# Vegeta2020/SE-SSD

Hardware: NVIDIA H100
Metric: frames_per_sec (higher is better)
Workload: dtype f32

## Files before the change

### include/sessd_b200_lab.h

```cpp
#ifndef SESSD_B200_LAB_H
#define SESSD_B200_LAB_H

#include "sessd_b200.h"

#ifdef __cplusplus
extern "C" {
#endif

int sessd_bev_conv_h2(const float *d_in, const void *d_weight_h2, int cout_pad, const float *d_scale,
                      const float *d_shift, const float *d_residual, float *d_out, const sessd_conv_desc *desc,
                      const float *d_amax_in, float *d_amax_out, void *stream);
int sessd_bev_deconv_h2(const float *d_in, const void *d_weight_h2, int cout_pad, const float *d_scale,
                        const float *d_shift, const float *d_residual, float *d_out, int batch, int in_h, int in_w,
                        int cin, int cout, int relu, const float *d_amax_in, float *d_amax_out, void *stream);

int sessd_bev_conv_p2_profile(const void *d_in_planes, const float *d_in_info, const void *d_weight_h2, int cout_pad,
                              const float *d_scale, const float *d_shift, const float *d_residual, const float *d_resid_info,
                              float gain, float shift_max, float *d_out_f32, void *d_out_planes, float *d_out_info,
                              const sessd_conv_desc *desc, const int *d_items, long long *d_prof, void *stream);
int sessd_bev_deconv_p2_profile(const void *d_in_planes, const float *d_in_info, const void *d_weight_h2, int cout_pad,
                                const float *d_scale, const float *d_shift, const float *d_residual, const float *d_resid_info,
                                float gain, float shift_max, float *d_out_f32, void *d_out_planes, float *d_out_info, int batch,
                                int in_h, int in_w, int cin, int cout, int relu, const int *d_items, long long *d_prof,
                                void *stream);

int sessd_bev_conv_p2_loads(const void *d_in_planes, const float *d_in_info, const void *d_weight_h2, int cout_pad,
                            const float *d_scale, const float *d_shift, const float *d_residual, const float *d_resid_info,
                            float gain, float shift_max, float *d_out_f32, void *d_out_planes, float *d_out_info,
                            const sessd_conv_desc *desc, const int *d_items, int smem_a, long long *d_prof, void *stream);

int sessd_bev_p2_plan(const sessd_conv_desc *desc, int deconv, int cout_pad, int split, int smem_a, int *plan);

#ifdef __cplusplus
}
#endif
#endif
```

### se-ssd_b200/csrc/bevconv_p2.cuh

```cuda
#pragma once
#include <cuda_fp16.h>

#include "tc_common.cuh"

namespace sessd {

constexpr int kP2TileU = 8, kP2TileV = 16;
constexpr int kP2MaxCopies = 6, kP2MaxRowsV = 18;
constexpr int kP2BStages = 6, kP2MaxBStages = 12;
constexpr int kP2MmaWarps = 8;
constexpr int kP2PatchWarp = 8, kP2WeightWarp = 9;
constexpr int kP2Threads = 320;
constexpr int kP2ThreadsRegA = 384, kP2RegsConsumer = 232, kP2RegsProducer = 40;
static_assert(2 * (kP2RegsConsumer - 168) <= 168 - kP2RegsProducer, "the consumers take what the producers release");
constexpr int kP2MaxSmem = 227 * 1024;
constexpr int kP2Chunk = 32;
constexpr int kP2ItemsHeader = 32;
enum { kP2Planes = 0, kP2SplitF16 = 1 };
enum { kP2NoProbe = 0, kP2ProbeClocks = 1, kP2ProbeLoads = 2 };

struct P2Params {
    int batch, cin, cout;
    int in_stride;
    int out_h, out_w;
    int grid_u, grid_v;
    int u_is_x;
    int out_stride, nclass;
    int cls_ntaps[4], cls_off_u[4], cls_off_v[4];
    int tap_copy[4][9], tap_row[4][9], tap_w[4][9];
    int ncopies, rows_v, pitch_u;
    int copy_u[kP2MaxCopies], copy_v[kP2MaxCopies];
    int copy_bytes, patch_bytes, npatch;
    int load_bytes, staging_bytes;
    int bring_bytes;
    int out_info_scale;
    const float *in_amax;
    int relu, n_tile, nblocks;
    int bstages, bstage_bytes;
    int tiles_u, tiles_v, tiles, total;
    int cls_order[4];
    const float *in_info;
    const float *resid_info;
    float gain, shift_max;
    float *out_info;
    long long out_plane_stride;
    const int *items;
    long long *prof;
};

// ... 78 lines not shown
        }
}

template <bool PROFILE>
__device__ __forceinline__ long long p2_tick() {
    if constexpr (PROFILE) return clock64();
    return 0;
}
template <bool PROFILE>
__device__ __forceinline__ void p2_tock(long long &clk, long long t0) {
    if constexpr (PROFILE) clk += clock64() - t0;
}

__device__ __forceinline__ void p2_split_patch(const P2Params &p, const unsigned char *staging, unsigned char *planes, float s_in, int ctid) {
    const int rows = p.rows_v * kP2TileU;
    const int copy_in = p.staging_bytes / p.ncopies;
    const int items = p.ncopies * rows * 4;
    for (int i = ctid; i < items; i += kP2MmaWarps * 32) {
        const int j = i & 3, r = (i >> 2) % rows, c = (i >> 2) / rows;
        unsigned char *hi = planes + 2 * c * p.copy_bytes + r * 64 + ((j ^ ((r >> 1) & 3)) << 4);
        const float4 *src = reinterpret_cast<const float4 *>(staging + c * copy_in + r * 128 + j * 32);
        const float4 a = src[0], b = src[1];
        const float x[8] = {a.x * s_in, a.y * s_in, a.z * s_in, a.w * s_in, b.x * s_in, b.y * s_in, b.z * s_in, b.w * s_in};
        __align__(16) __half h[8], l[8];
#pragma unroll
        for (int t = 0; t < 8; ++t) { h[t] = __float2half_rn(x[t]); l[t] = __float2half_rn(x[t] - __half2float(h[t])); }
        *reinterpret_cast<uint4 *>(hi) = *reinterpret_cast<const uint4 *>(h);
        *reinterpret_cast<uint4 *>(hi + p.copy_bytes) = *reinterpret_cast<const uint4 *>(l);
    }
    asm volatile("fence.proxy.async.shared::cta;\n" ::: "memory");
    asm volatile("bar.sync 1, %0;\n" ::"n"(kP2MmaWarps * 32) : "memory");
}

template <int NT, int MODE, bool REGA = false, int PROBE = kP2NoProbe>
__global__ void __launch_bounds__(REGA ? kP2ThreadsRegA : kP2Threads, 1) bev_conv_p2_kernel(const __grid_constant__ CUtensorMap map_a,
                                                                   const __grid_constant__ CUtensorMap map_b,
                                                                   const float *__restrict__ scale, const float *__restrict__ shift,
                                                                   const float *__restrict__ resid, float *__restrict__ out_f32,
                                                                   __half *__restrict__ out_planes, P2Params p) {
    static_assert(!REGA || MODE == kP2Planes, "register-fed A reads the TMA-written planes");
    constexpr bool PROFILE = PROBE != kP2NoProbe, LOADS_ONLY = PROBE == kP2ProbeLoads;
    extern __shared__ unsigned char smem_raw[];
    unsigned char *tiles = (unsigned char *)(((uintptr_t)smem_raw + 1023) & ~(uintptr_t)1023);
    unsigned char *patches = tiles + p.bring_bytes;
    unsigned char *staging = patches + p.npatch * p.patch_bytes;
    uint64_t *bars = (uint64_t *)(staging + p.npatch * p.staging_bytes);
    uint64_t *patch_full = bars, *patch_empty = bars + 2, *b_full = bars + 4, *b_empty = bars + 4 + kP2MaxBStages;
    uint32_t *s_aoff = (uint32_t *)(b_empty + kP2MaxBStages);
    float *s_scale = (float *)(((uintptr_t)(s_aoff + 4 * 9) + 15) & ~(uintptr_t)15), *s_shift = s_scale + p.cout;

    const int warp = threadIdx.x >> 5, lane = threadIdx.x & 31;
    if (threadIdx.x == kP2PatchWarp * 32) prefetch_tensormap(&map_a);
    if (threadIdx.x == kP2WeightWarp * 32) prefetch_tensormap(&map_b);
    const int nchunks = p.cin / kP2Chunk;
    const int nitems = p2_item_count(p);
    const uint32_t b_plane_bytes = (uint32_t)p.n_tile * 64u;

    if (threadIdx.x == 0) {
        for (int s = 0; s < 2; ++s) { mbar_init(&patch_full[s], 1); mbar_init(&patch_empty[s], kP2MmaWarps); }
        for (int s = 0; s < p.bstages; ++s) { mbar_init(&b_full[s], 1); mbar_init(&b_empty[s], kP2MmaWarps); }
        asm volatile("fence.mbarrier_init.release.cluster;\n" ::: "memory");
    }
    for (int idx = threadIdx.x; idx < p.nclass * 9; idx += blockDim.x) {
        const int c = idx / 9, t = idx - c * 9;
        s_aoff[idx] = REGA ? (uint32_t)p.tap_row[c][t] : (uint32_t)((2 * p.tap_copy[c][t] * p.copy_bytes + p.tap_row[c][t] * 512) >> 4);
    }
    for (int n = threadIdx.x; n < p.cout; n += blockDim.x) {
        s_scale[n] = scale ? __ldg(scale + n) : 1.f;
        s_shift[n] = shift ? __ldg(shift + n) : 0.f;
    }
    __syncthreads();
    long long clk[kP2ProfWords] = {};
    const long long t_start = p2_tick<PROFILE>();
    long long *prof_rec = PROFILE ? p.prof + (size_t)blockIdx.x * kP2ProfWords : nullptr;

    if (warp >= kP2MmaWarps) {
        if constexpr (REGA) setmaxnreg_dec<kP2RegsProducer>();
        if (warp == kP2PatchWarp) {
            int pb = 0;
            uint32_t pph = 0;
            const uint32_t patches_u32 = smem_u32(patches);
            for (int k = blockIdx.x; k < nitems; k += gridDim.x) {
                const P2Item it = p2_decode(p, p2_item(p, k));
                const int bu = it.u0 * p.in_stride, bv = it.v0 * p.in_stride;
                for (int cc = 0; cc < nchunks; ++cc) {
                    { const long long t0 = p2_tick<PROFILE>(); mbar_wait<REGA>(&patch_empty[pb], pph ^ 1u); p2_tock<PROFILE>(clk[kProfPatchEmpty], t0); }
                    if (elect_one()) {
                        mbar_expect_tx(&patch_full[pb], (uint32_t)p.load_bytes);
                        if constexpr (MODE == kP2Planes) {
                            uint32_t dst = patches_u32 + (uint32_t)(pb * p.patch_bytes);
                            for (int c = 0; c < p.ncopies; ++c, dst += 2u * (uint32_t)p.copy_bytes) {
                                const int cu = bu + p.copy_u[c], cv = bv + p.copy_v[c];
                                tma_load_5d(dst, &map_a, &patch_full[pb], cc * kP2Chunk, cu, cv, it.b, 0);
                                tma_load_5d(dst + (uint32_t)p.copy_bytes, &map_a, &patch_full[pb], cc * kP2Chunk, cu, cv, it.b, 1);
                            }
                        } else {
                            const uint32_t copy_in = (uint32_t)(p.staging_bytes / p.ncopies);
                            uint32_t dst = smem_u32(staging) + (uint32_t)(pb * p.staging_bytes);
                            for (int c = 0; c < p.ncopies; ++c, dst += copy_in)
                                tma_load_5d(dst, &map_a, &patch_full[pb], cc * kP2Chunk, bu + p.copy_u[c], bv + p.copy_v[c], it.b, 0);
                        }
                    }
                    __syncwarp();
                    if (++pb == p.npatch) { pb = 0; pph ^= 1u; }
                }
            }
            if constexpr (PROFILE)
                if (lane == 0) {
                    prof_rec[kProfPatchEmpty] = clk[kProfPatchEmpty];
                    prof_rec[kProfPatchTotal] = clock64() - t_start;
                }
        } else if (warp == kP2WeightWarp) {
            int S = 0;
            uint32_t bph = 0;
            for (int k = blockIdx.x; k < nitems; k += gridDim.x) {
                const P2Item it = p2_decode(p, p2_item(p, k));
                for (int cc = 0; cc < nchunks; ++cc)
                    for (int tap = 0; tap < it.ntaps; ++tap) {
// ... 24 lines not shown
        const uint32_t patch_lo = desc_lo(smem_u32(patches)) + a_rows;
        const uint32_t plane_lo = b_plane_bytes >> 4;
        const uint32_t copy_lo = (uint32_t)(p.copy_bytes >> 4), patch_sz = (uint32_t)(p.patch_bytes >> 4);
        const uint32_t a_row = (uint32_t)((wg * 8 + wq * 2 + ((lane >> 3) & 1)) * p.pitch_u + (lane & 7)), a_chunk = (uint32_t)(lane >> 4);
        const uint32_t patches_u32 = smem_u32(patches);
        float amax_in = 0.f, s_in = 1.f;
        if constexpr (MODE == kP2Planes) { amax_in = __ldg(p.in_info); s_in = __ldg(p.in_info + 1); }
        if constexpr (MODE == kP2SplitF16) if (p.in_amax) { amax_in = __ldg(p.in_amax); s_in = pow2_scale_for_bound(amax_in); }
        const float inv_sa = 1.f / s_in;
        float bound = amax_in * p.gain + p.shift_max;
        if (p.resid_info) bound += __ldg(p.resid_info);
        const float s_out = pow2_scale_for_bound(bound);
        if (blockIdx.x == 0 && threadIdx.x == 0 && p.out_info && p.out_info_scale) p.out_info[1] = s_out;
        float vmax = 0.f;
        const int per_cls = p.nblocks * p.tiles;
        int S = 0, pb = 0;
        uint32_t bph = 0, pph = 0;
        for (int k = blockIdx.x; k < nitems; k += gridDim.x) {
            const long long t_item = p2_tick<PROFILE>();
            const int g = p2_item(p, k);
            const int cls = p.cls_order[g / per_cls];
            const int ntaps = p.cls_ntaps[cls];
            const uint32_t *aoff = s_aoff + cls * 9;
            float acc[NT];
#pragma unroll
            for (int i = 0; i < NT; ++i) acc[i] = 0.f;
            int prevS = -1, prev_pb = -1;
            bool first = true;
            if constexpr (REGA) {
                uint32_t frag[2][16];
                int tap = 0;
                uint32_t pbase = 0;
                auto load_frags = [&](uint32_t *fa) {
                    if (tap == 0) {
                        { const long long t0 = p2_tick<PROFILE>(); mbar_wait<REGA>(&patch_full[pb], pph); p2_tock<PROFILE>(clk[kProfPatchFull], t0); }
                        pbase = patches_u32 + (uint32_t)(pb * p.patch_bytes);
                    }
                    if constexpr (!LOADS_ONLY) {
                        const uint32_t r = a_row + aoff[tap];
                        const uint32_t a_hi = pbase + r * 64u + ((a_chunk ^ ((r >> 1) & 3u)) << 4), a_lo = a_hi + (uint32_t)p.copy_bytes;
                        ldsm_x4(fa, a_hi);
                        ldsm_x4(fa + 4, a_hi ^ 32u);
                        ldsm_x4(fa + 8, a_lo);
                        ldsm_x4(fa + 12, a_lo ^ 32u);
                    }
                };
                auto step_ra = [&](const uint32_t *fa, uint32_t *fn, bool more) {
                    { const long long t0 = p2_tick<PROFILE>(); mbar_wait<REGA>(&b_full[S], bph); p2_tock<PROFILE>(clk[kProfBFull], t0); }
                    const uint64_t db_lo = kDescSw64Hi | (uint64_t)(tiles_lo + (uint32_t)(S * (p.bstage_bytes >> 4)));
                    const uint64_t db_hi = db_lo + (uint64_t)plane_lo;
                    if constexpr (!LOADS_ONLY) {
                        wgmma_fence();
                        p2_wgmma_ra<2 * NT>(acc, fa, db_lo, first ? 0u : 1u);
                        p2_wgmma_ra<2 * NT>(acc, fa + 4, db_lo + 2, 1u);
                        wgmma_commit();
                    }
                    first = false;
                    if constexpr (PROFILE) ++clk[kProfSteps];
                    { const long long t0 = p2_tick<PROFILE>(); wgmma_wait<1>(); p2_tock<PROFILE>(clk[kProfMmaWait], t0); }
                    if (lane == 0 && prevS >= 0) mbar_arrive(&b_empty[prevS]);
                    prevS = S;
                    if (++S == p.bstages) { S = 0; bph ^= 1u; }
                    if (++tap == ntaps) {
                        tap = 0;
                        if (lane == 0) mbar_arrive(&patch_empty[pb]);
                        if (++pb == p.npatch) { pb = 0; pph ^= 1u; }
                    }
                    if (more) load_frags(fn);
                    if constexpr (!LOADS_ONLY) {
                        wgmma_fence();
                        p2_wgmma_ra<NT>(acc, fa + 8, db_hi, 1u);
                        p2_wgmma_ra<NT>(acc, fa + 12, db_hi + 2, 1u);
                        wgmma_commit();
                    }
                };
                const int nsteps = nchunks * ntaps;
                load_frags(frag[0]);
#pragma unroll 1
                for (int st = 0; st + 1 < nsteps; st += 2) { step_ra(frag[0], frag[1], true); step_ra(frag[1], frag[0], st + 2 < nsteps); }
                if (nsteps & 1) step_ra(frag[0], frag[1], false);
            } else {
                for (int cc = 0; cc < nchunks; ++cc) {
                    { const long long t0 = p2_tick<PROFILE>(); mbar_wait(&patch_full[pb], pph); p2_tock<PROFILE>(clk[kProfPatchFull], t0); }
                    if constexpr (MODE == kP2SplitF16)
                        p2_split_patch(p, staging + pb * p.staging_bytes, patches + pb * p.patch_bytes, s_in, threadIdx.x);
                    const uint32_t pbase = patch_lo + (uint32_t)pb * patch_sz;
#pragma unroll 1
                    for (int tap = 0; tap < ntaps; ++tap) {
                        { const long long t0 = p2_tick<PROFILE>(); mbar_wait(&b_full[S], bph); p2_tock<PROFILE>(clk[kProfBFull], t0); }
                        if constexpr (!LOADS_ONLY) {
                            const uint64_t da_hi = kDescSw64Hi | (uint64_t)(pbase + aoff[tap]);
                            const uint64_t da_lo = da_hi + (uint64_t)copy_lo;
                            const uint64_t db_lo = kDescSw64Hi | (uint64_t)(tiles_lo + (uint32_t)(S * (p.bstage_bytes >> 4)));
                            const uint64_t db_hi = db_lo + (uint64_t)plane_lo;
                            const uint32_t accum = first ? 0u : 1u;
                            wgmma_fence();
                            if constexpr (MODE == kP2Planes) {
                                p2_wgmma<2 * NT>(acc, da_hi, db_lo, accum);
// ... 161 lines not shown
constexpr int p2_n_tile(int cout) { return cout <= 32 ? 32 : 128; }

struct P2Geometry {
    int u_is_x, grid_u, grid_v, tiles_u, tiles_v, tiles;
    int n_tile, nblocks, nclass, total;
    int ntaps[4], off_u[4], off_v[4], order[4];
};

static int p2_geometry(P2Geometry &g, int batch, int grid_h, int grid_w, int cout, int cout_pad, const P2Taps *cls, int nclass) {
    g = {};
    if (batch < 1 || grid_h < 1 || grid_w < 1 || cout < 8 || cout % 8) return SESSD_EINVAL;
    g.n_tile = p2_n_tile(cout);
    if (cout_pad % g.n_tile || cout_pad < cout) return SESSD_EINVAL;
    g.u_is_x = div_up(grid_w, kP2TileU) * div_up(grid_h, kP2TileV) <= div_up(grid_h, kP2TileU) * div_up(grid_w, kP2TileV);
    g.grid_u = g.u_is_x ? grid_w : grid_h; g.grid_v = g.u_is_x ? grid_h : grid_w;
    g.tiles_u = div_up(g.grid_u, kP2TileU); g.tiles_v = div_up(g.grid_v, kP2TileV);
    g.tiles = g.tiles_u * g.tiles_v * batch;
    g.nblocks = cout_pad / g.n_tile;
    g.nclass = nclass; g.total = nclass * g.nblocks * g.tiles;
    for (int c = 0; c < nclass; ++c) {
        g.ntaps[c] = cls[c].n;
        g.off_u[c] = g.u_is_x ? cls[c].off_x : cls[c].off_y;
        g.off_v[c] = g.u_is_x ? cls[c].off_y : cls[c].off_x;
        g.order[c] = c;
    }
    for (int i = 1; i < nclass; ++i)
        for (int k = i; k > 0 && g.ntaps[g.order[k]] > g.ntaps[g.order[k - 1]]; --k) {
            const int tmp = g.order[k]; g.order[k] = g.order[k - 1]; g.order[k - 1] = tmp;
        }
    return 0;
}

static int p2_plan(P2Params &p, const P2Taps *cls, int nclass, int grid_h, int grid_w, int cout_pad, int mode, bool reg_a, int *smem) {
    if (reg_a && (mode != kP2Planes || p.in_stride != 1)) return SESSD_EINVAL;
    if (p.cin < 64 || p.cin % 64) return SESSD_EINVAL;
    P2Geometry g;
    if (p2_geometry(g, p.batch, grid_h, grid_w, p.cout, cout_pad, cls, nclass)) return SESSD_EINVAL;
    p.u_is_x = g.u_is_x; p.grid_u = g.grid_u; p.grid_v = g.grid_v;
    p.tiles_u = g.tiles_u; p.tiles_v = g.tiles_v; p.tiles = g.tiles;
    p.n_tile = g.n_tile; p.nblocks = g.nblocks; p.nclass = g.nclass; p.total = g.total;
    for (int c = 0; c < 4; ++c) {
        p.cls_ntaps[c] = g.ntaps[c]; p.cls_off_u[c] = g.off_u[c]; p.cls_off_v[c] = g.off_v[c]; p.cls_order[c] = g.order[c];
    }
    const int s = p.in_stride;
    p.ncopies = 0;
    int key_u[kP2MaxCopies], key_vm[kP2MaxCopies], vmin[kP2MaxCopies], vmax[kP2MaxCopies];
    for (int c = 0; c < p.nclass; ++c)
        for (int t = 0; t < cls[c].n; ++t) {
            const int tu = p.u_is_x ? cls[c].dx[t] : cls[c].dy[t], tv = p.u_is_x ? cls[c].dy[t] : cls[c].dx[t];
            const int vm = ((tv % s) + s) % s;
            int k = 0;
            for (; k < p.ncopies; ++k)
                if (key_u[k] == tu && key_vm[k] == vm) break;
            if (k == p.ncopies) {
                if (p.ncopies == kP2MaxCopies) return SESSD_EINVAL;
                key_u[k] = tu; key_vm[k] = vm; vmin[k] = tv; vmax[k] = tv;
                ++p.ncopies;
            }
            vmin[k] = min(vmin[k], tv); vmax[k] = max(vmax[k], tv);
        }
    p.rows_v = 0;
    p.pitch_u = kP2TileU;
    for (int k = 0; k < p.ncopies; ++k) p.rows_v = max(p.rows_v, kP2TileV + (vmax[k] - vmin[k]) / s);
    if (p.rows_v > kP2MaxRowsV) return SESSD_EINVAL;
    for (int k = 0; k < p.ncopies; ++k) { p.copy_u[k] = key_u[k]; p.copy_v[k] = vmin[k]; }
    if (reg_a) {
        int umin = key_u[0], umax = key_u[0];
        for (int k = 1; k < p.ncopies; ++k) {
            umin = min(umin, key_u[k]); umax = max(umax, key_u[k]);
            vmin[0] = min(vmin[0], vmin[k]); vmax[0] = max(vmax[0], vmax[k]);
        }
        p.ncopies = 1;
        p.copy_u[0] = umin; p.copy_v[0] = vmin[0];
        p.pitch_u = kP2TileU + umax - umin; p.rows_v = kP2TileV + vmax[0] - vmin[0];
        if (p.pitch_u > 256 || p.rows_v > 256) return SESSD_EINVAL;
    }
    for (int c = 0; c < p.nclass; ++c) {
        for (int t = 0; t < cls[c].n; ++t) {
            const int tu = p.u_is_x ? cls[c].dx[t] : cls[c].dy[t], tv = p.u_is_x ? cls[c].dy[t] : cls[c].dx[t];
            const int vm = ((tv % s) + s) % s;
            int k = 0;
            for (; k < p.ncopies; ++k)
                if (key_u[k] == tu && key_vm[k] == vm) break;
            p.tap_copy[c][t] = reg_a ? 0 : k;
            p.tap_row[c][t] = reg_a ? (tv - p.copy_v[0]) * p.pitch_u + (tu - p.copy_u[0]) : (tv - vmin[k]) / s;
            p.tap_w[c][t] = cls[c].w[t];
        }
    }
    p.copy_bytes = (p.rows_v * p.pitch_u * 64 + 511) & ~511;
    p.patch_bytes = p.ncopies * 2 * p.copy_bytes;
    p.staging_bytes = mode == kP2Planes ? 0 : p.ncopies * p.rows_v * kP2TileU * kP2Chunk * 4;
    p.load_bytes = mode == kP2Planes ? p.ncopies * 2 * p.rows_v * p.pitch_u * 64 : p.staging_bytes;
    const int per_buf = p.patch_bytes + p.staging_bytes, bstage = 2 * p.n_tile * 64;
    const int tail = 1536 + 16 + 2 * 4 * p.cout;
    p.npatch = (kP2BStages * bstage + tail + 2 * per_buf <= kP2MaxSmem) ? 2 : 1;
    p.bstage_bytes = bstage;
    p.bstages = min((kP2MaxSmem - tail - p.npatch * per_buf) / bstage, kP2MaxBStages);
    if (p.bstages < 2) return SESSD_EINVAL;
    p.bring_bytes = p.bstages * bstage;
    *smem = p.bring_bytes + tail + p.npatch * per_buf;
    return 0;
}

template <int MODE, int PROBE = kP2NoProbe>
static int launch_p2(const void *d_in_planes, int in_h, int in_w, const float *d_in_info, const void *d_w, int w_taps, int cout_pad,
                     const float *d_scale, const float *d_shift, const float *d_residual, const float *d_resid_info, float gain,
                     float shift_max, float *d_out_f32, void *d_out_planes, float *d_out_info, P2Params &p, const P2Taps *cls, int nclass,
                     int grid_h, int grid_w, bool reg_a, void *stream) {
    if (!d_in_planes || !d_w || (!d_out_f32 && !d_out_planes)) return SESSD_EINVAL;
    if (MODE == kP2Planes && (!d_in_info || !d_scale)) return SESSD_EINVAL;
    if (MODE != kP2Planes && d_out_planes) return SESSD_EINVAL;
    if (((uintptr_t)d_scale | (uintptr_t)d_shift | (uintptr_t)d_residual | (uintptr_t)d_out_f32 | (uintptr_t)d_out_planes) & 15)
        return SESSD_EINVAL;
    int smem = 0;
    if (p2_plan(p, cls, nclass, grid_h, grid_w, cout_pad, MODE, reg_a, &smem)) return SESSD_EINVAL;
    if (p.items && cout_pad != div_up(p.cout, p.n_tile) * p.n_tile) return SESSD_EINVAL;
    const int s = p.in_stride;
    CUtensorMap map_a, map_b;
    if (MODE != kP2Planes) {
        const cuuint64_t row_w = (cuuint64_t)p.cin * 4, row_h = (cuuint64_t)in_w * p.cin * 4;
        const cuuint64_t dims[5] = {(cuuint64_t)p.cin, (cuuint64_t)(p.u_is_x ? in_w : in_h), (cuuint64_t)(p.u_is_x ? in_h : in_w),
                                    (cuuint64_t)p.batch, 1};
        const cuuint64_t strides[4] = {p.u_is_x ? row_w : row_h, p.u_is_x ? row_h : row_w, (cuuint64_t)in_h * in_w * p.cin * 4,
                                       (cuuint64_t)p.batch * in_h * in_w * p.cin * 4};
        const cuuint32_t box[5] = {(cuuint32_t)kP2Chunk, (cuuint32_t)(kP2TileU * s), (cuuint32_t)(p.rows_v * s), 1, 1};
        const cuuint32_t estr[5] = {1, (cuuint32_t)s, (cuuint32_t)s, 1, 1};
        int rc = encode_map_nd(&map_a, d_in_planes, 5, dims, strides, box, estr, CU_TENSOR_MAP_SWIZZLE_NONE, CU_TENSOR_MAP_DATA_TYPE_FLOAT32);
        if (rc) return rc;
    } else {
        const cuuint64_t row_w = (cuuint64_t)p.cin * 2, row_h = (cuuint64_t)in_w * p.cin * 2;
        const cuuint64_t dims[5] = {(cuuint64_t)p.cin, (cuuint64_t)(p.u_is_x ? in_w : in_h), (cuuint64_t)(p.u_is_x ? in_h : in_w),
                                    (cuuint64_t)p.batch, 2};
        const cuuint64_t strides[4] = {p.u_is_x ? row_w : row_h, p.u_is_x ? row_h : row_w, (cuuint64_t)in_h * in_w * p.cin * 2,
                                       (cuuint64_t)p.batch * in_h * in_w * p.cin * 2};
        const cuuint32_t box[5] = {(cuuint32_t)kP2Chunk, (cuuint32_t)(p.pitch_u * s), (cuuint32_t)(p.rows_v * s), 1, 1};
        const cuuint32_t estr[5] = {1, (cuuint32_t)s, (cuuint32_t)s, 1, 1};
        int rc = encode_map_nd(&map_a, d_in_planes, 5, dims, strides, box, estr, CU_TENSOR_MAP_SWIZZLE_64B);
        if (rc) return rc;
    }
    {
        const cuuint64_t dims[4] = {(cuuint64_t)p.cin, (cuuint64_t)cout_pad, (cuuint64_t)w_taps, 2};
        const cuuint64_t strides[3] = {(cuuint64_t)p.cin * 2, (cuuint64_t)cout_pad * p.cin * 2, (cuuint64_t)w_taps * cout_pad * p.cin * 2};
        const cuuint32_t box[4] = {(cuuint32_t)kP2Chunk, (cuuint32_t)p.n_tile, 1, 1};
        const cuuint32_t estr[4] = {1, 1, 1, 1};
        int rc = encode_map_nd(&map_b, d_w, 4, dims, strides, box, estr, CU_TENSOR_MAP_SWIZZLE_64B);
        if (rc) return rc;
    }
    constexpr bool kRegA = MODE == kP2Planes;
    auto kernel = bev_conv_p2_kernel<128, MODE, false, PROBE>;
    if (p.n_tile == 32) kernel = reg_a ? bev_conv_p2_kernel<32, MODE, kRegA, PROBE> : bev_conv_p2_kernel<32, MODE, false, PROBE>;
    else if (reg_a) kernel = bev_conv_p2_kernel<128, MODE, kRegA, PROBE>;
    static bool attr_done[2][2] = {};
    if (!attr_done[p.n_tile == 32][reg_a]) {
        SESSD_CUDA_TRY(cudaFuncSetAttribute(kernel, cudaFuncAttributeMaxDynamicSharedMemorySize, kP2MaxSmem));
        attr_done[p.n_tile == 32][reg_a] = true;
    }
    p.in_info = MODE == kP2Planes ? d_in_info : nullptr;
    p.in_amax = MODE == kP2SplitF16 ? d_in_info : nullptr;
    p.resid_info = d_residual ? d_resid_info : nullptr;
    if (d_residual && d_out_planes && !d_resid_info) return SESSD_EINVAL;
    p.gain = gain; p.shift_max = shift_max; p.out_info = d_out_info;
    p.out_info_scale = MODE == kP2Planes ? 1 : 0;
    if (d_out_planes && !d_out_info) return SESSD_EINVAL;
    p.out_plane_stride = (long long)p.batch * p.out_h * p.out_w * p.cout;
    static int num_sms = 0;
    if (!num_sms) {
        int dev = 0;
        SESSD_CUDA_TRY(cudaGetDevice(&dev));
        SESSD_CUDA_TRY(cudaDeviceGetAttribute(&num_sms, cudaDevAttrMultiProcessorCount, dev));
    }
    const int grid = p.total < num_sms ? p.total : num_sms;
    SESSD_LAUNCH(kernel, grid, reg_a ? kP2ThreadsRegA : kP2Threads, smem, (cudaStream_t)stream, map_a, map_b, d_scale, d_shift, d_residual, d_out_f32,
                 (__half *)d_out_planes, p);
    return last_error();
}


static int p2_conv_params(const sessd_conv_desc &d, P2Params &p, P2Taps &t) {
    if (d.ntaps < 1 || d.ntaps > 9 || (d.in_stride != 1 && d.in_stride != 2) || d.out_stride < 1) return SESSD_EINVAL;
    if ((d.grid_h - 1) * d.out_stride + d.out_off_y >= d.out_h || (d.grid_w - 1) * d.out_stride + d.out_off_x >= d.out_w) return SESSD_EINVAL;
    p = {};
    p.batch = d.batch; p.cin = d.cin; p.cout = d.cout; p.in_stride = d.in_stride;
    p.out_h = d.out_h; p.out_w = d.out_w; p.out_stride = d.out_stride; p.relu = d.relu;
    t = {};
    t.n = d.ntaps; t.off_y = d.out_off_y; t.off_x = d.out_off_x;
    for (int i = 0; i < d.ntaps; ++i) { t.dy[i] = d.tap_dy[i]; t.dx[i] = d.tap_dx[i]; t.w[i] = i; }
    return 0;
}

static void p2_deconv_params(int batch, int in_h, int in_w, int cin, int cout, int relu, P2Params &p, P2Taps cls[4]) {
    p = {};
    p.batch = batch; p.cin = cin; p.cout = cout; p.in_stride = 1;
    p.out_h = 2 * in_h; p.out_w = 2 * in_w; p.out_stride = 2; p.relu = relu;
    p2_deconv_classes(cls);
}

template <int MODE, int PROBE = kP2NoProbe>
static int p2_conv(const void *d_in_planes, const float *d_in_info, const void *d_weight_h2, int cout_pad, const float *d_scale,
                   const float *d_shift, const float *d_residual, const float *d_resid_info, float gain, float shift_max,
                   float *d_out_f32, void *d_out_planes, float *d_out_info, const sessd_conv_desc *desc, void *stream,
                   const int *d_items = nullptr, long long *d_prof = nullptr, bool smem_a = false) {
    if (!desc || (PROBE != kP2NoProbe && !d_prof)) return SESSD_EINVAL;
    const sessd_conv_desc &d = *desc;
    P2Params p;
    P2Taps t;
    if (p2_conv_params(d, p, t)) return SESSD_EINVAL;
    p.items = d_items;
    p.prof = d_prof;
    return launch_p2<MODE, PROBE>(d_in_planes, d.in_h, d.in_w, d_in_info, d_weight_h2, d.ntaps, cout_pad, d_scale, d_shift, d_residual, d_resid_info, gain,
                     shift_max, d_out_f32, d_out_planes, d_out_info, p, &t, 1, d.grid_h, d.grid_w, MODE == kP2Planes && d.in_stride == 1 && !smem_a,
                     stream);
}

template <int MODE, int PROBE = kP2NoProbe>
static int p2_deconv(const void *d_in_planes, const float *d_in_info, const void *d_weight_h2, int cout_pad, const float *d_scale,
                     const float *d_shift, const float *d_residual, const float *d_resid_info, float gain, float shift_max,
                     float *d_out_f32, void *d_out_planes, float *d_out_info, int batch, int in_h, int in_w, int cin, int cout,
                     int relu, void *stream, const int *d_items = nullptr, long long *d_prof = nullptr) {
    if (PROBE != kP2NoProbe && !d_prof) return SESSD_EINVAL;
    P2Params p;
    P2Taps cls[4];
    p2_deconv_params(batch, in_h, in_w, cin, cout, relu, p, cls);
    p.items = d_items;
    p.prof = d_prof;
    return launch_p2<MODE, PROBE>(d_in_planes, in_h, in_w, d_in_info, d_weight_h2, 9, cout_pad, d_scale, d_shift, d_residual, d_resid_info, gain, shift_max,
                     d_out_f32, d_out_planes, d_out_info, p, cls, 4, in_h, in_w, MODE == kP2Planes, stream);
}

}
```

### se-ssd_b200/csrc/bevconv_split.cu

```cuda
#include "bevconv_p2.cuh"

#include "../../include/sessd_b200_lab.h"

using namespace sessd;

extern "C" int sessd_bev_conv_h2(const float *d_in, const void *d_weight_h2, int cout_pad, const float *d_scale, const float *d_shift,
                                 const float *d_residual, float *d_out, const sessd_conv_desc *desc, const float *d_amax_in,
                                 float *d_amax_out, void *stream) {
    if (!d_in || !d_out || !d_scale) return SESSD_EINVAL;
    return p2_conv<kP2SplitF16>(d_in, d_amax_in, d_weight_h2, cout_pad, d_scale, d_shift, d_residual, nullptr, 0.f, 0.f, d_out, nullptr,
                                d_amax_out, desc, stream);
}

extern "C" int sessd_bev_deconv_h2(const float *d_in, const void *d_weight_h2, int cout_pad, const float *d_scale, const float *d_shift,
                                   const float *d_residual, float *d_out, int batch, int in_h, int in_w, int cin, int cout, int relu,
                                   const float *d_amax_in, float *d_amax_out, void *stream) {
    if (!d_in || !d_out || !d_scale) return SESSD_EINVAL;
    return p2_deconv<kP2SplitF16>(d_in, d_amax_in, d_weight_h2, cout_pad, d_scale, d_shift, d_residual, nullptr, 0.f, 0.f, d_out, nullptr,
                                  d_amax_out, batch, in_h, in_w, cin, cout, relu, stream);
}

extern "C" int sessd_bev_conv_p2_profile(const void *d_in_planes, const float *d_in_info, const void *d_weight_h2, int cout_pad,
                                         const float *d_scale, const float *d_shift, const float *d_residual, const float *d_resid_info,
                                         float gain, float shift_max, float *d_out_f32, void *d_out_planes, float *d_out_info,
                                         const sessd_conv_desc *desc, const int *d_items, long long *d_prof, void *stream) {
    return p2_conv<kP2Planes, kP2ProbeClocks>(d_in_planes, d_in_info, d_weight_h2, cout_pad, d_scale, d_shift, d_residual, d_resid_info, gain,
                                              shift_max, d_out_f32, d_out_planes, d_out_info, desc, stream, d_items, d_prof);
}

extern "C" int sessd_bev_deconv_p2_profile(const void *d_in_planes, const float *d_in_info, const void *d_weight_h2, int cout_pad,
                                           const float *d_scale, const float *d_shift, const float *d_residual, const float *d_resid_info,
                                           float gain, float shift_max, float *d_out_f32, void *d_out_planes, float *d_out_info, int batch,
                                           int in_h, int in_w, int cin, int cout, int relu, const int *d_items, long long *d_prof,
                                           void *stream) {
    return p2_deconv<kP2Planes, kP2ProbeClocks>(d_in_planes, d_in_info, d_weight_h2, cout_pad, d_scale, d_shift, d_residual, d_resid_info, gain,
                                                shift_max, d_out_f32, d_out_planes, d_out_info, batch, in_h, in_w, cin, cout, relu, stream,
                                                d_items, d_prof);
}

extern "C" int sessd_bev_conv_p2_loads(const void *d_in_planes, const float *d_in_info, const void *d_weight_h2, int cout_pad,
                                       const float *d_scale, const float *d_shift, const float *d_residual, const float *d_resid_info,
                                       float gain, float shift_max, float *d_out_f32, void *d_out_planes, float *d_out_info,
                                       const sessd_conv_desc *desc, const int *d_items, int smem_a, long long *d_prof, void *stream) {
    return p2_conv<kP2Planes, kP2ProbeLoads>(d_in_planes, d_in_info, d_weight_h2, cout_pad, d_scale, d_shift, d_residual, d_resid_info, gain,
                                             shift_max, d_out_f32, d_out_planes, d_out_info, desc, stream, d_items, d_prof, smem_a != 0);
}

extern "C" int sessd_bev_p2_plan(const sessd_conv_desc *desc, int deconv, int cout_pad, int split, int smem_a, int *plan) {
    if (!desc || !plan) return SESSD_EINVAL;
    const sessd_conv_desc &d = *desc;
    P2Params p;
    P2Taps cls[4];
    if (deconv) p2_deconv_params(d.batch, d.in_h, d.in_w, d.cin, d.cout, d.relu, p, cls);
    else if (p2_conv_params(d, p, cls[0])) return SESSD_EINVAL;
    const int mode = split ? kP2SplitF16 : kP2Planes;
    const bool reg_a = mode == kP2Planes && (deconv || (d.in_stride == 1 && !smem_a));
    int smem = 0;
    if (p2_plan(p, cls, deconv ? 4 : 1, deconv ? d.in_h : d.grid_h, deconv ? d.in_w : d.grid_w, cout_pad, mode, reg_a, &smem))
        return SESSD_EINVAL;
    const int rec[11] = {p.u_is_x, p.n_tile, p.nblocks, p.tiles, p.total, p.ncopies, p.rows_v, p.pitch_u, p.npatch, p.bstages, smem};
    for (int i = 0; i < 11; ++i) plan[i] = rec[i];
    for (int c = 0; c < 4; ++c) { plan[11 + c] = p.cls_ntaps[c]; plan[15 + c] = p.cls_order[c]; }
    return 0;
}
```

### se-ssd_b200/sessd_b200/_lib.py

```python
import ctypes as C
import os

_HERE = os.path.dirname(os.path.abspath(__file__))
LIB_PATH = os.path.join(os.path.dirname(_HERE), "libsessd_b200.so")
LAB_PATH = os.path.join(os.path.dirname(_HERE), "libsessd_b200_lab.so")


class SessdError(RuntimeError):
    pass


class VoxelCfg(C.Structure):
    _fields_ = [("voxel_size", C.c_float * 3), ("range_min", C.c_float * 3), ("range_max", C.c_float * 3),
                ("grid", C.c_int * 3), ("max_points", C.c_int), ("max_voxels", C.c_int), ("num_feat", C.c_int)]


class Grid(C.Structure):
    _fields_ = [("batch", C.c_int), ("shape", C.c_int * 3)]


class ConvDesc(C.Structure):
    _fields_ = [("batch", C.c_int), ("in_h", C.c_int), ("in_w", C.c_int), ("cin", C.c_int),
                ("out_h", C.c_int), ("out_w", C.c_int), ("cout", C.c_int),
                ("grid_h", C.c_int), ("grid_w", C.c_int), ("in_stride", C.c_int),
# ... 69 lines not shown
    "sessd_rotate_nms": (_i, [_vp, _vp, _vp, _i, _i, _i, _f, _i, _vp, _vp, _vp, _sz, _vp]),
    "sessd_boxes_overlap_bev": (_i, [_vp, _i, _vp, _i, _vp, _vp]),
    "sessd_boxes_aligned_overlap_bev": (_i, [_vp, _vp, _i, _vp, _vp]),
    "sessd_boxes_iou_bev": (_i, [_vp, _i, _vp, _i, _vp, _vp]),
    "sessd_boxes_iou3d": (_i, [_vp, _i, _vp, _i, _vp, _vp]),
    "sessd_nms_workspace_bytes": (_sz, [_i]),
    "sessd_nms_sorted": (_i, [_vp, _i, _f, _i, _vp, _vp, _vp, _sz, _vp]),
    "sessd_head_loss_workspace_bytes": (_sz, [_i]),
    "sessd_head_loss": (_i, [_vp, _vp, _vp, _vp, _i, _i, _i, _i, _f, _f, _f, _f, _f, _f, _f, _f, _vp, _vp, _vp, _sz, _vp]),
    "sessd_odiou_loss_workspace_bytes": (_sz, [_i]),
    "sessd_odiou_loss": (_i, [_vp, _vp, _vp, _vp, _i, _i, _i, _i, _f, _vp, _vp, _vp, _vp, _sz, _vp]),
    "sessd_odiou_pairs_host": (_i, [_vp, _vp, _i, _vp, _vp]),
    "sessd_iou_pred_loss_workspace_bytes": (_sz, [_i]),
    "sessd_iou_pred_loss": (_i, [_vp, _vp, _vp, _vp, _i, _i, _i, _i, _f, _f, _vp, _vp, _vp, _sz, _vp]),
    "sessd_axpby": (_i, [_vp, _vp, _f, _f, _ll, _vp]),
    "sessd_adamw_step": (_i, [_vp, _vp, _vp, _vp, _ll, _f, _f, _f, _f, _f, _i, _vp]),
    "sessd_grad_sqnorm_workspace_bytes": (_sz, [_ll]),
    "sessd_grad_sqnorm": (_i, [_vp, _ll, _f, _vp, _vp, _vp]),
    "sessd_adamw_clip_ema_step": (_i, [_vp, _vp, _vp, _vp, _ll, _f, _f, _f, _f, _f, _i, _vp, _vp, C.c_double, _vp]),
    "sessd_assign_workspace_bytes": (_sz, [_i, _i, _i]),
    "sessd_assign_targets": (_i, [_vp, _i, _vp, _vp, _i, _i, _f, _f, _vp, _vp, _vp, _vp, _vp, _vp, _vp, _sz, _vp]),
    "sessd_kitti_convert_workspace_bytes": (_sz, [_ll]),
    "sessd_kitti_convert_detections": (_i, [_vp, _vp, _vp, _vp, _i, _ll, _vp, _vp, _vp, _i, _vp, _vp, _vp, _vp, _vp, _sz, _vp]),
    "sessd_kitti_overlaps": (_i, [C.POINTER(KittiFrames), _i, _i, C.c_double, _vp, _vp]),
    "sessd_kitti_eval_workspace_bytes": (_sz, [_i, _ll, _ll, _i, _i]),
    "sessd_kitti_eval": (_i, [C.POINTER(KittiFrames), _i, _i, _i, C.c_double, _i, _vp, _vp, _i, _ll, _ll, _vp, _vp, _vp, _vp, _vp, _vp,
                              _sz, _vp]),
}


LAB_SIGNATURES = {
    "sessd_bev_conv_h2": (_i, [_vp, _vp, _i, _vp, _vp, _vp, _vp, C.POINTER(ConvDesc), _vp, _vp, _vp]),
    "sessd_bev_deconv_h2": (_i, [_vp, _vp, _i, _vp, _vp, _vp, _vp, _i, _i, _i, _i, _i, _i, _vp, _vp, _vp]),
    "sessd_bev_conv_p2_profile": (_i, [_vp, _vp, _vp, _i, _vp, _vp, _vp, _vp, _f, _f, _vp, _vp, _vp, C.POINTER(ConvDesc), _vp, _vp, _vp]),
    "sessd_bev_deconv_p2_profile": (_i, [_vp, _vp, _vp, _i, _vp, _vp, _vp, _vp, _f, _f, _vp, _vp, _vp, _i, _i, _i, _i, _i, _i, _vp, _vp,
                                         _vp]),
    "sessd_bev_conv_p2_loads": (_i, [_vp, _vp, _vp, _i, _vp, _vp, _vp, _vp, _f, _f, _vp, _vp, _vp, C.POINTER(ConvDesc), _vp, _i, _vp, _vp]),
    "sessd_bev_p2_plan": (_i, [C.POINTER(ConvDesc), _i, _i, _i, _i, _I3]),
}


def _load(path, signatures, mode=C.DEFAULT_MODE):
    if not os.path.exists(path):
        raise ImportError(
            "sessd_b200: %s is missing -- the CUDA library has not been built (run `python se-ssd_b200/build.py`). "
            "There is no CPU fallback." % path)
    lib = C.CDLL(path, mode=mode)
    for name, (res, args) in signatures.items():
        fn = getattr(lib, name)
        fn.restype = res
        fn.argtypes = args
    return lib


class _Libs:

    def __init__(self):
        self._prod = _load(LIB_PATH, SIGNATURES, C.RTLD_GLOBAL)
        self._lab = None

    def lab(self):
        if self._lab is None:
            self._lab = _load(LAB_PATH, LAB_SIGNATURES)
        return self._lab

    @property
    def lab_loaded(self):
# ... 24 lines not shown
```

Baseline: 1396.

## Extend register-fed A path to strided convs with per-copy patch barriers

Allows the register-fed A variant for strided convolutions, placing multiple input copies in the patch buffer with per-copy row offsets. Adds a COPYWISE kernel variant in which each copy gets its own full/empty mbarrier pair. Consumers wait only for the copy a tap needs and release it after its last tap, so MMA can start before every copy has landed. This adds more barriers and per-tap bit decoding, and shifts the strided convs onto a different kernel configuration.

```diff
diff --git a/include/sessd_b200_lab.h b/include/sessd_b200_lab.h
--- a/include/sessd_b200_lab.h
+++ b/include/sessd_b200_lab.h
@@ -17,7 +17,7 @@
 int sessd_bev_conv_p2_profile(const void *d_in_planes, const float *d_in_info, const void *d_weight_h2, int cout_pad,
                               const float *d_scale, const float *d_shift, const float *d_residual, const float *d_resid_info,
                               float gain, float shift_max, float *d_out_f32, void *d_out_planes, float *d_out_info,
-                              const sessd_conv_desc *desc, const int *d_items, long long *d_prof, void *stream);
+                              const sessd_conv_desc *desc, const int *d_items, int smem_a, long long *d_prof, void *stream);
 int sessd_bev_deconv_p2_profile(const void *d_in_planes, const float *d_in_info, const void *d_weight_h2, int cout_pad,
                                 const float *d_scale, const float *d_shift, const float *d_residual, const float *d_resid_info,
                                 float gain, float shift_max, float *d_out_f32, void *d_out_planes, float *d_out_info, int batch,
diff --git a/se-ssd_b200/csrc/bevconv_p2.cuh b/se-ssd_b200/csrc/bevconv_p2.cuh
--- a/se-ssd_b200/csrc/bevconv_p2.cuh
+++ b/se-ssd_b200/csrc/bevconv_p2.cuh
@@ -15,6 +15,8 @@
 static_assert(2 * (kP2RegsConsumer - 168) <= 168 - kP2RegsProducer, "the consumers take what the producers release");
 constexpr int kP2MaxSmem = 227 * 1024;
 constexpr int kP2Chunk = 32;
+constexpr uint32_t kP2TapRowMask = 0xFFFFFFu, kP2TapFirst = 1u << 28, kP2TapLast = 1u << 29;
+__host__ __device__ constexpr uint32_t p2_tap_copy(uint32_t e) { return (e >> 24) & 15u; }
 constexpr int kP2ItemsHeader = 32;
 enum { kP2Planes = 0, kP2SplitF16 = 1 };
 enum { kP2NoProbe = 0, kP2ProbeClocks = 1, kP2ProbeLoads = 2 };
@@ -159,20 +161,22 @@
     asm volatile("bar.sync 1, %0;\n" ::"n"(kP2MmaWarps * 32) : "memory");
 }
 
-template <int NT, int MODE, bool REGA = false, int PROBE = kP2NoProbe>
+template <int NT, int MODE, bool REGA = false, int PROBE = kP2NoProbe, bool COPYWISE = false>
 __global__ void __launch_bounds__(REGA ? kP2ThreadsRegA : kP2Threads, 1) bev_conv_p2_kernel(const __grid_constant__ CUtensorMap map_a,
                                                                    const __grid_constant__ CUtensorMap map_b,
                                                                    const float *__restrict__ scale, const float *__restrict__ shift,
                                                                    const float *__restrict__ resid, float *__restrict__ out_f32,
                                                                    __half *__restrict__ out_planes, P2Params p) {
     static_assert(!REGA || MODE == kP2Planes, "register-fed A reads the TMA-written planes");
+    static_assert(!COPYWISE || REGA, "copy-by-copy patches are read from registers");
     constexpr bool PROFILE = PROBE != kP2NoProbe, LOADS_ONLY = PROBE == kP2ProbeLoads;
     extern __shared__ unsigned char smem_raw[];
     unsigned char *tiles = (unsigned char *)(((uintptr_t)smem_raw + 1023) & ~(uintptr_t)1023);
     unsigned char *patches = tiles + p.bring_bytes;
     unsigned char *staging = patches + p.npatch * p.patch_bytes;
     uint64_t *bars = (uint64_t *)(staging + p.npatch * p.staging_bytes);
-    uint64_t *patch_full = bars, *patch_empty = bars + 2, *b_full = bars + 4, *b_empty = bars + 4 + kP2MaxBStages;
+    constexpr int kPatchBars = COPYWISE ? kP2MaxCopies : 2;
+    uint64_t *patch_full = bars, *patch_empty = bars + kPatchBars, *b_full = bars + 2 * kPatchBars, *b_empty = b_full + kP2MaxBStages;
     uint32_t *s_aoff = (uint32_t *)(b_empty + kP2MaxBStages);
     float *s_scale = (float *)(((uintptr_t)(s_aoff + 4 * 9) + 15) & ~(uintptr_t)15), *s_shift = s_scale + p.cout;
 
@@ -184,13 +188,22 @@
     const uint32_t b_plane_bytes = (uint32_t)p.n_tile * 64u;
 
     if (threadIdx.x == 0) {
-        for (int s = 0; s < 2; ++s) { mbar_init(&patch_full[s], 1); mbar_init(&patch_empty[s], kP2MmaWarps); }
+        for (int s = 0; s < kPatchBars; ++s) { mbar_init(&patch_full[s], 1); mbar_init(&patch_empty[s], kP2MmaWarps); }
         for (int s = 0; s < p.bstages; ++s) { mbar_init(&b_full[s], 1); mbar_init(&b_empty[s], kP2MmaWarps); }
         asm volatile("fence.mbarrier_init.release.cluster;\n" ::: "memory");
     }
     for (int idx = threadIdx.x; idx < p.nclass * 9; idx += blockDim.x) {
-        const int c = idx / 9, t = idx - c * 9;
-        s_aoff[idx] = REGA ? (uint32_t)p.tap_row[c][t] : (uint32_t)((2 * p.tap_copy[c][t] * p.copy_bytes + p.tap_row[c][t] * 512) >> 4);
+        const int c = idx / 9, t = idx - c * 9, k = p.tap_copy[c][t];
+        if constexpr (COPYWISE) {
+            bool first = true, last = true;
+            for (int u = 0; u < p.cls_ntaps[c]; ++u)
+                if (p.tap_copy[c][u] == k) { first &= !(u < t); last &= !(u > t); }
+            s_aoff[idx] = (uint32_t)p.tap_row[c][t] | ((uint32_t)k << 24) | (first ? kP2TapFirst : 0u) | (last ? kP2TapLast : 0u);
+        } else if constexpr (REGA) {
+            s_aoff[idx] = (uint32_t)p.tap_row[c][t];
+        } else {
+            s_aoff[idx] = (uint32_t)((2 * k * p.copy_bytes + p.tap_row[c][t] * 512) >> 4);
+        }
     }
     for (int n = threadIdx.x; n < p.cout; n += blockDim.x) {
         s_scale[n] = scale ? __ldg(scale + n) : 1.f;
@@ -211,6 +224,22 @@
                 const P2Item it = p2_decode(p, p2_item(p, k));
                 const int bu = it.u0 * p.in_stride, bv = it.v0 * p.in_stride;
                 for (int cc = 0; cc < nchunks; ++cc) {
+                    if constexpr (COPYWISE) {
+                        const uint32_t copy_load = (uint32_t)(p.load_bytes / p.ncopies);
+                        uint32_t dst = patches_u32;
+                        for (int c = 0; c < p.ncopies; ++c, dst += 2u * (uint32_t)p.copy_bytes) {
+                            { const long long t0 = p2_tick<PROFILE>(); mbar_wait<REGA>(&patch_empty[c], pph ^ 1u); p2_tock<PROFILE>(clk[kProfPatchEmpty], t0); }
+                            if (elect_one()) {
+                                const int cu = bu + p.copy_u[c], cv = bv + p.copy_v[c];
+                                mbar_expect_tx(&patch_full[c], copy_load);
+                                tma_load_5d(dst, &map_a, &patch_full[c], cc * kP2Chunk, cu, cv, it.b, 0);
+                                tma_load_5d(dst + (uint32_t)p.copy_bytes, &map_a, &patch_full[c], cc * kP2Chunk, cu, cv, it.b, 1);
+                            }
+                            __syncwarp();
+                        }
+                        pph ^= 1u;
+                        continue;
+                    }
                     { const long long t0 = p2_tick<PROFILE>(); mbar_wait<REGA>(&patch_empty[pb], pph ^ 1u); p2_tock<PROFILE>(clk[kProfPatchEmpty], t0); }
                     if (elect_one()) {
                         mbar_expect_tx(&patch_full[pb], (uint32_t)p.load_bytes);
@@ -301,12 +330,13 @@
                 int tap = 0;
                 uint32_t pbase = 0;
                 auto load_frags = [&](uint32_t *fa) {
-                    if (tap == 0) {
-                        { const long long t0 = p2_tick<PROFILE>(); mbar_wait<REGA>(&patch_full[pb], pph); p2_tock<PROFILE>(clk[kProfPatchFull], t0); }
+                    if (COPYWISE ? (aoff[tap] & kP2TapFirst) != 0u : tap == 0) {
+                        const int slot = COPYWISE ? (int)p2_tap_copy(aoff[tap]) : pb;
+                        { const long long t0 = p2_tick<PROFILE>(); mbar_wait<REGA>(&patch_full[slot], pph); p2_tock<PROFILE>(clk[kProfPatchFull], t0); }
                         pbase = patches_u32 + (uint32_t)(pb * p.patch_bytes);
                     }
                     if constexpr (!LOADS_ONLY) {
-                        const uint32_t r = a_row + aoff[tap];
+                        const uint32_t r = a_row + (COPYWISE ? aoff[tap] & kP2TapRowMask : aoff[tap]);
                         const uint32_t a_hi = pbase + r * 64u + ((a_chunk ^ ((r >> 1) & 3u)) << 4), a_lo = a_hi + (uint32_t)p.copy_bytes;
                         ldsm_x4(fa, a_hi);
                         ldsm_x4(fa + 4, a_hi ^ 32u);
@@ -330,9 +360,11 @@
                     if (lane == 0 && prevS >= 0) mbar_arrive(&b_empty[prevS]);
                     prevS = S;
                     if (++S == p.bstages) { S = 0; bph ^= 1u; }
+                    if constexpr (COPYWISE)
+                        if (lane == 0 && (aoff[tap] & kP2TapLast)) mbar_arrive(&patch_empty[p2_tap_copy(aoff[tap])]);
                     if (++tap == ntaps) {
                         tap = 0;
-                        if (lane == 0) mbar_arrive(&patch_empty[pb]);
+                        if (!COPYWISE && lane == 0) mbar_arrive(&patch_empty[pb]);
                         if (++pb == p.npatch) { pb = 0; pph ^= 1u; }
                     }
                     if (more) load_frags(fn);
@@ -560,7 +592,7 @@
 }
 
 static int p2_plan(P2Params &p, const P2Taps *cls, int nclass, int grid_h, int grid_w, int cout_pad, int mode, bool reg_a, int *smem) {
-    if (reg_a && (mode != kP2Planes || p.in_stride != 1)) return SESSD_EINVAL;
+    if (reg_a && mode != kP2Planes) return SESSD_EINVAL;
     if (p.cin < 64 || p.cin % 64) return SESSD_EINVAL;
     P2Geometry g;
     if (p2_geometry(g, p.batch, grid_h, grid_w, p.cout, cout_pad, cls, nclass)) return SESSD_EINVAL;
@@ -592,7 +624,8 @@
     for (int k = 0; k < p.ncopies; ++k) p.rows_v = max(p.rows_v, kP2TileV + (vmax[k] - vmin[k]) / s);
     if (p.rows_v > kP2MaxRowsV) return SESSD_EINVAL;
     for (int k = 0; k < p.ncopies; ++k) { p.copy_u[k] = key_u[k]; p.copy_v[k] = vmin[k]; }
-    if (reg_a) {
+    const bool one_copy = reg_a && s == 1;
+    if (one_copy) {
         int umin = key_u[0], umax = key_u[0];
         for (int k = 1; k < p.ncopies; ++k) {
             umin = min(umin, key_u[k]); umax = max(umax, key_u[k]);
@@ -603,6 +636,7 @@
         p.pitch_u = kP2TileU + umax - umin; p.rows_v = kP2TileV + vmax[0] - vmin[0];
         if (p.pitch_u > 256 || p.rows_v > 256) return SESSD_EINVAL;
     }
+    p.copy_bytes = (p.rows_v * p.pitch_u * 64 + 511) & ~511;
     for (int c = 0; c < p.nclass; ++c) {
         for (int t = 0; t < cls[c].n; ++t) {
             const int tu = p.u_is_x ? cls[c].dx[t] : cls[c].dy[t], tv = p.u_is_x ? cls[c].dy[t] : cls[c].dx[t];
@@ -610,12 +644,12 @@
             int k = 0;
             for (; k < p.ncopies; ++k)
                 if (key_u[k] == tu && key_vm[k] == vm) break;
-            p.tap_copy[c][t] = reg_a ? 0 : k;
-            p.tap_row[c][t] = reg_a ? (tv - p.copy_v[0]) * p.pitch_u + (tu - p.copy_u[0]) : (tv - vmin[k]) / s;
+            if (one_copy) k = 0;
+            p.tap_copy[c][t] = k;
+            p.tap_row[c][t] = reg_a ? 2 * k * p.copy_bytes / 64 + (tv - p.copy_v[k]) / s * p.pitch_u + (tu - p.copy_u[k]) : (tv - vmin[k]) / s;
             p.tap_w[c][t] = cls[c].w[t];
         }
     }
-    p.copy_bytes = (p.rows_v * p.pitch_u * 64 + 511) & ~511;
     p.patch_bytes = p.ncopies * 2 * p.copy_bytes;
     p.staging_bytes = mode == kP2Planes ? 0 : p.ncopies * p.rows_v * kP2TileU * kP2Chunk * 4;
     p.load_bytes = mode == kP2Planes ? p.ncopies * 2 * p.rows_v * p.pitch_u * 64 : p.staging_bytes;
@@ -675,13 +709,18 @@
         if (rc) return rc;
     }
     constexpr bool kRegA = MODE == kP2Planes;
+    const bool copywise = reg_a && p.npatch == 1 && p.nclass == 1 && p.ncopies > 1;
     auto kernel = bev_conv_p2_kernel<128, MODE, false, PROBE>;
-    if (p.n_tile == 32) kernel = reg_a ? bev_conv_p2_kernel<32, MODE, kRegA, PROBE> : bev_conv_p2_kernel<32, MODE, false, PROBE>;
-    else if (reg_a) kernel = bev_conv_p2_kernel<128, MODE, kRegA, PROBE>;
-    static bool attr_done[2][2] = {};
-    if (!attr_done[p.n_tile == 32][reg_a]) {
+    if (p.n_tile == 32)
+        kernel = !reg_a ? bev_conv_p2_kernel<32, MODE, false, PROBE>
+                        : copywise ? bev_conv_p2_kernel<32, MODE, kRegA, PROBE, kRegA> : bev_conv_p2_kernel<32, MODE, kRegA, PROBE>;
+    else if (reg_a)
+        kernel = copywise ? bev_conv_p2_kernel<128, MODE, kRegA, PROBE, kRegA> : bev_conv_p2_kernel<128, MODE, kRegA, PROBE>;
+    const int variant = reg_a + copywise;
+    static bool attr_done[2][3] = {};
+    if (!attr_done[p.n_tile == 32][variant]) {
         SESSD_CUDA_TRY(cudaFuncSetAttribute(kernel, cudaFuncAttributeMaxDynamicSharedMemorySize, kP2MaxSmem));
-        attr_done[p.n_tile == 32][reg_a] = true;
+        attr_done[p.n_tile == 32][variant] = true;
     }
     p.in_info = MODE == kP2Planes ? d_in_info : nullptr;
     p.in_amax = MODE == kP2SplitF16 ? d_in_info : nullptr;
@@ -736,8 +775,7 @@
     p.items = d_items;
     p.prof = d_prof;
     return launch_p2<MODE, PROBE>(d_in_planes, d.in_h, d.in_w, d_in_info, d_weight_h2, d.ntaps, cout_pad, d_scale, d_shift, d_residual, d_resid_info, gain,
-                     shift_max, d_out_f32, d_out_planes, d_out_info, p, &t, 1, d.grid_h, d.grid_w, MODE == kP2Planes && d.in_stride == 1 && !smem_a,
-                     stream);
+                     shift_max, d_out_f32, d_out_planes, d_out_info, p, &t, 1, d.grid_h, d.grid_w, MODE == kP2Planes && !smem_a, stream);
 }
 
 template <int MODE, int PROBE = kP2NoProbe>
diff --git a/se-ssd_b200/csrc/bevconv_split.cu b/se-ssd_b200/csrc/bevconv_split.cu
--- a/se-ssd_b200/csrc/bevconv_split.cu
+++ b/se-ssd_b200/csrc/bevconv_split.cu
@@ -23,9 +23,9 @@
 extern "C" int sessd_bev_conv_p2_profile(const void *d_in_planes, const float *d_in_info, const void *d_weight_h2, int cout_pad,
                                          const float *d_scale, const float *d_shift, const float *d_residual, const float *d_resid_info,
                                          float gain, float shift_max, float *d_out_f32, void *d_out_planes, float *d_out_info,
-                                         const sessd_conv_desc *desc, const int *d_items, long long *d_prof, void *stream) {
+                                         const sessd_conv_desc *desc, const int *d_items, int smem_a, long long *d_prof, void *stream) {
     return p2_conv<kP2Planes, kP2ProbeClocks>(d_in_planes, d_in_info, d_weight_h2, cout_pad, d_scale, d_shift, d_residual, d_resid_info, gain,
-                                              shift_max, d_out_f32, d_out_planes, d_out_info, desc, stream, d_items, d_prof);
+                                              shift_max, d_out_f32, d_out_planes, d_out_info, desc, stream, d_items, d_prof, smem_a != 0);
 }
 
 extern "C" int sessd_bev_deconv_p2_profile(const void *d_in_planes, const float *d_in_info, const void *d_weight_h2, int cout_pad,
@@ -54,7 +54,7 @@
     if (deconv) p2_deconv_params(d.batch, d.in_h, d.in_w, d.cin, d.cout, d.relu, p, cls);
     else if (p2_conv_params(d, p, cls[0])) return SESSD_EINVAL;
     const int mode = split ? kP2SplitF16 : kP2Planes;
-    const bool reg_a = mode == kP2Planes && (deconv || (d.in_stride == 1 && !smem_a));
+    const bool reg_a = mode == kP2Planes && (deconv || !smem_a);
     int smem = 0;
     if (p2_plan(p, cls, deconv ? 4 : 1, deconv ? d.in_h : d.grid_h, deconv ? d.in_w : d.grid_w, cout_pad, mode, reg_a, &smem))
         return SESSD_EINVAL;
diff --git a/se-ssd_b200/sessd_b200/_lib.py b/se-ssd_b200/sessd_b200/_lib.py
--- a/se-ssd_b200/sessd_b200/_lib.py
+++ b/se-ssd_b200/sessd_b200/_lib.py
@@ -125,7 +125,7 @@
 LAB_SIGNATURES = {
     "sessd_bev_conv_h2": (_i, [_vp, _vp, _i, _vp, _vp, _vp, _vp, C.POINTER(ConvDesc), _vp, _vp, _vp]),
     "sessd_bev_deconv_h2": (_i, [_vp, _vp, _i, _vp, _vp, _vp, _vp, _i, _i, _i, _i, _i, _i, _vp, _vp, _vp]),
-    "sessd_bev_conv_p2_profile": (_i, [_vp, _vp, _vp, _i, _vp, _vp, _vp, _vp, _f, _f, _vp, _vp, _vp, C.POINTER(ConvDesc), _vp, _vp, _vp]),
+    "sessd_bev_conv_p2_profile": (_i, [_vp, _vp, _vp, _i, _vp, _vp, _vp, _vp, _f, _f, _vp, _vp, _vp, C.POINTER(ConvDesc), _vp, _i, _vp, _vp]),
     "sessd_bev_deconv_p2_profile": (_i, [_vp, _vp, _vp, _i, _vp, _vp, _vp, _vp, _f, _f, _vp, _vp, _vp, _i, _i, _i, _i, _i, _i, _vp, _vp,
                                          _vp]),
     "sessd_bev_conv_p2_loads": (_i, [_vp, _vp, _vp, _i, _vp, _vp, _vp, _vp, _f, _f, _vp, _vp, _vp, C.POINTER(ConvDesc), _vp, _i, _vp, _vp]),
```

New measurement: 1402, median of 6. About the same (+0.4%).
